# Lynne-Zheng-Linfang/HS-Pose

Measured on AMD Instinct MI355X. Metric: point-clouds/sec (N=1028) HS-layer fwd+bwd, higher is better.
Workload: dtype f32; 1 GPU; HS stack (FaceRecon backbone -> feat) fwd+bwd, B=16/GPU N=1028 fp32, train-mode BN, random-init weights (BASELINE configs[1] shape); global_batch=16, points=1028, parallelism=dp1, hipgraph=True, split_graph=False, grad_exchange=none

## Files before the change

hs_pose_amd/csrc/gather.hip:

```cpp
#include "common.h"
#include "colsum_cloud.h"
#include <type_traits>

namespace hsp {

template <typename FT>
__device__ __forceinline__ void gather_max_rows(const FT* __restrict__ fb, const int32_t* __restrict__ nb, int k,
                                                int C, float4& best, int& a0, int& a1, int& a2, int& a3) {
    constexpr int NB = 8;
    int cur[NB], nxt[NB];
#pragma unroll
    for (int u = 0; u < NB; ++u) cur[u] = nb[min(u, k - 1)];
    for (int n0 = 0; n0 < k; n0 += NB) {
#pragma unroll
        for (int u = 0; u < NB; ++u) nxt[u] = nb[min(n0 + NB + u, k - 1)];
        float4 f[NB];
#pragma unroll
        for (int u = 0; u < NB; ++u) f[u] = Feat<FT>::ld4(fb + (size_t)cur[u] * C);
#pragma unroll
        for (int u = 0; u < NB; ++u) {
            const int n = n0 + u;
            if (n < k) {
                if (f[u].x > best.x) { best.x = f[u].x; a0 = n; }
                if (f[u].y > best.y) { best.y = f[u].y; a1 = n; }
// ... 288 lines not shown
            for (int l = 1; l < RL; ++l) { const float4 v = red[q][l * cq + g]; a.x += v.x; a.y += v.y; a.z += v.z; a.w += v.w; }
            *reinterpret_cast<float4*>(part + (((size_t)b * nchunk + chunk) * 4 + q) * C + (g << 2)) = a;
        }
    }
}

template <bool XYZ>
__global__ __launch_bounds__(1024) void colsum_cloud_kernel(const float* __restrict__ x, const float* __restrict__ xyz, int N, int C,
                                                            int nchunk, int rows, float* __restrict__ out) {
    extern __shared__ float4 cc_smem[];
    colsum_cloud_body<XYZ, 1024, 1>(cc_smem, (int)blockIdx.x, (int)blockIdx.y, x, xyz, N, C, nchunk, rows, out);
}

__global__ __launch_bounds__(256) void colsum_partial_scalar_kernel(const float* __restrict__ x, int N, int C,
                                                                    float* __restrict__ part, int nchunk, int rows) {
    __shared__ float red[256];
    const int tid = threadIdx.x;
    const int RL = 256 / C;
    const int col = tid % C, rl = tid / C;
    const int b = blockIdx.y, chunk = blockIdx.x;
    const int r0 = chunk * rows, r1 = min(N, r0 + rows);
    float s = 0.f;
    if (rl < RL)
        for (int i = r0 + rl; i < r1; i += RL) s += x[((size_t)b * N + i) * C + col];
    red[tid] = s;
    __syncthreads();
    if (rl == 0) {
        for (int l = 1; l < RL; ++l) s += red[l * C + col];
        part[((size_t)b * nchunk + chunk) * C + col] = s;
    }
}

struct ConcatSeg { const void* src; const int32_t* idx; int width; int kind; int nsrc; int col0; };
struct ConcatDesc { ConcatSeg seg[8]; int nseg; int even; int q0[9]; };

template <typename FT>
__global__ __launch_bounds__(256) void concat_rows_kernel(ConcatDesc d, int B, int N, int W, FT* __restrict__ out) {
    using Pair = typename std::conditional<sizeof(FT) == 4, float2, unsigned>::type;
    const long long rows = (long long)B * N;
    if (d.even == 2) {
        const int lane = threadIdx.x & 63;
        const int total = d.q0[d.nseg];
        for (long long row = (long long)blockIdx.x * 4 + (threadIdx.x >> 6); row < rows; row += (long long)gridDim.x * 4) {
            const int b = (int)(row / N);
            FT* o = out + (size_t)row * W;
            for (int q = lane; q < total; q += 64) {
                int sgi = 0;
                while (q >= d.q0[sgi + 1]) ++sgi;
                const ConcatSeg sg = d.seg[sgi];
                const int c = q - d.q0[sgi];
                if (sg.kind >= 2) {
                    const float* ps = reinterpret_cast<const float*>(sg.src);
                    Feat<FT>::st(o + sg.col0 + c, sg.kind == 2 ? ps[(size_t)b * sg.width + c] : ((long long)ps[b] == c ? 1.f : 0.f));
                    continue;
                }
                const FT* src = reinterpret_cast<const FT*>(sg.src);
                src += sg.kind == 0 ? (size_t)row * sg.width : ((size_t)b * sg.nsrc + sg.idx[row]) * sg.width;
                reinterpret_cast<uint4*>(o + sg.col0)[c] = reinterpret_cast<const uint4*>(src)[c];
            }
            const int used = d.seg[d.nseg - 1].col0 + d.seg[d.nseg - 1].width;
            if (lane < W - used) Feat<FT>::st(o + used + lane, 0.f);
        }
        return;
    }
    for (long long row = blockIdx.x; row < rows; row += gridDim.x) {
        const int b = (int)(row / N);
        FT* o = out + (size_t)row * W;
        for (int s = 0; s < d.nseg; ++s) {
            const ConcatSeg sg = d.seg[s];
            if (sg.kind >= 2) {
                const float* src = reinterpret_cast<const float*>(sg.src);
                for (int c = threadIdx.x; c < sg.width; c += 256)
                    Feat<FT>::st(o + sg.col0 + c, sg.kind == 2 ? src[(size_t)b * sg.width + c] : ((long long)src[b] == c ? 1.f : 0.f));
                continue;
            }
            const FT* src = reinterpret_cast<const FT*>(sg.src);
            if (sg.kind == 0) src += (size_t)row * sg.width;
            else src += ((size_t)b * sg.nsrc + sg.idx[row]) * sg.width;
            if (d.even) {
                const Pair* s2 = reinterpret_cast<const Pair*>(src);
                Pair* o2 = reinterpret_cast<Pair*>(o + sg.col0);
                for (int c = threadIdx.x; c < (sg.width >> 1); c += 256) o2[c] = s2[c];
            } else {
                for (int c = threadIdx.x; c < sg.width; c += 256) o[sg.col0 + c] = src[c];
            }
        }
    }
}

__global__ __launch_bounds__(256) void gather_max_bwd_kernel(const float* __restrict__ gout, int gbcast,
                                                             const int32_t* __restrict__ idx,
                                                             const int32_t* __restrict__ qsel, int qstride,
                                                             const uint8_t* __restrict__ argmax, int B, int Nsrc,
                                                             int Nidx, int Nq, int kstride, int C,
                                                             float* __restrict__ gfeat) {
    const int cq = C >> 2;
    const long long total = (long long)B * Nq * cq;
// ... 509 lines not shown
extern "C" int hsp_gather_rows_fwd(const float* feat, const int32_t* idx, int idx_shared, int B, int Nsrc, int Nq,
                                   int C, float* out, int out_stride, hspStream_t stream) {
    if (!feat || !idx || !out || B <= 0 || Nsrc <= 0 || Nq <= 0 || C <= 0 || out_stride < C) return HSP_ERR_BAD_ARG;
    hipStream_t st = as_stream(stream);
    if ((C & 3) == 0) {
        const long long total = (long long)B * Nq * (C >> 2);
        hipLaunchKernelGGL(gather_rows_fwd_kernel, dim3(stream_grid(total)), dim3(256), 0, st, feat, idx, idx_shared, B,
                           Nsrc, Nq, C, out, out_stride);
    } else {
        const long long total = (long long)B * Nq * C;
        hipLaunchKernelGGL(gather_rows_fwd_scalar_kernel, dim3(stream_grid(total)), dim3(256), 0, st, feat, idx,
                           idx_shared, B, Nsrc, Nq, C, out, out_stride);
    }
    return check_launch();
}

extern "C" int hsp_gather_rows_bwd(const float* grad_out, int grad_stride, const int32_t* idx, int idx_shared, int B,
                                   int Nsrc, int Nq, int C, float* grad_feat, hspStream_t stream) {
    if (!grad_out || !idx || !grad_feat || B <= 0 || Nsrc <= 0 || Nq <= 0 || C <= 0 || grad_stride < C)
        return HSP_ERR_BAD_ARG;
    hipStream_t st = as_stream(stream);
    if ((C & 3) == 0 && (grad_stride & 1) == 0 && (reinterpret_cast<uintptr_t>(grad_out) & 7) == 0)
        if (const int tc = pick_scatter_cols(Nsrc, C))
            return launch_scatter_tile<1, float>(tc, grad_out, nullptr, grad_stride, 0, idx, idx_shared, nullptr, 0, nullptr, B,
                                                 Nsrc, Nq, Nq, 1, C, grad_feat, 0, nullptr, st);
    hipError_t e = hipMemsetAsync(grad_feat, 0, (size_t)B * Nsrc * C * sizeof(float), st);
    if (e != hipSuccess) { set_last_hip_error(e); return HSP_ERR_LAUNCH; }
    const long long total = (long long)B * Nq * C;
    hipLaunchKernelGGL(gather_rows_bwd_kernel, dim3(stream_grid(total)), dim3(256), 0, st, grad_out, grad_stride, idx,
                       idx_shared, B, Nsrc, Nq, C, grad_feat);
    return check_launch();
}

template <typename FT, int VEC>
__device__ __forceinline__ void grow_ld(const FT* __restrict__ p, float (&v)[VEC]) {
    if constexpr (sizeof(FT) == 4 && VEC == 2) {
        const float2 t = *reinterpret_cast<const float2*>(p);
        v[0] = t.x; v[1] = t.y;
    } else if constexpr (sizeof(FT) == 4) {
        const float4 t = *reinterpret_cast<const float4*>(p);
        v[0] = t.x; v[1] = t.y; v[2] = t.z; v[3] = t.w;
    } else if constexpr (VEC == 2) {
        const unsigned w = *reinterpret_cast<const unsigned*>(p);
        v[0] = __uint_as_float(w << 16); v[1] = __uint_as_float(w & 0xffff0000u);
    } else {
        const uint2 w = *reinterpret_cast<const uint2*>(p);
        v[0] = __uint_as_float(w.x << 16); v[1] = __uint_as_float(w.x & 0xffff0000u);
        v[2] = __uint_as_float(w.y << 16); v[3] = __uint_as_float(w.y & 0xffff0000u);
    }
}
template <typename FT, int VEC>
__device__ __forceinline__ void grow_st(FT* __restrict__ p, const float (&v)[VEC]) {
    if constexpr (sizeof(FT) == 4 && VEC == 2) {
        *reinterpret_cast<float2*>(p) = make_float2(v[0], v[1]);
    } else if constexpr (sizeof(FT) == 4) {
        *reinterpret_cast<float4*>(p) = make_float4(v[0], v[1], v[2], v[3]);
    } else if constexpr (VEC == 2) {
        *reinterpret_cast<unsigned*>(p) = f32_to_bf16_bits(v[0]) | (f32_to_bf16_bits(v[1]) << 16);
    } else {
        *reinterpret_cast<uint2*>(p) = make_uint2(f32_to_bf16_bits(v[0]) | (f32_to_bf16_bits(v[1]) << 16),
                                                  f32_to_bf16_bits(v[2]) | (f32_to_bf16_bits(v[3]) << 16));
    }
}

template <typename FT, int VEC>
__device__ __forceinline__ void gather_rows_bwd_csr_body(const int bid, const FT* __restrict__ gout, int gstride,
                                                         const int32_t* __restrict__ rev_off,
                                                         const int32_t* __restrict__ rev_edge, int B, int Nsrc, int Nq, int C,
                                                         FT* __restrict__ gfeat) {
    const int cols = C / VEC;
    const int tpr = cols < 256 ? cols : 256;
    const int RB = 256 / tpr;
    const int rl = threadIdx.x / tpr, t = threadIdx.x - rl * tpr;
    const long long row = (long long)bid * RB + rl;
    if (rl >= RB || row >= (long long)B * Nsrc) return;
    const int m = (int)(row % Nsrc), b = (int)(row / Nsrc);
    const int32_t* off = rev_off + (size_t)b * (Nsrc + 1);
    const int32_t* edge = rev_edge + (size_t)b * Nq;
    const int o0 = off[m], o1 = off[m + 1];
    const FT* gb = gout + (size_t)b * Nq * gstride;
    for (int p = t; p < cols; p += tpr) {
        float acc[VEC];
#pragma unroll
        for (int c = 0; c < VEC; ++c) acc[c] = 0.f;
        int e = o0;
        for (; e + 8 <= o1; e += 8) {
            float v[8][VEC];
#pragma unroll
            for (int u = 0; u < 8; ++u) grow_ld<FT, VEC>(gb + (size_t)edge[e + u] * gstride + VEC * p, v[u]);
// ... 16 lines not shown
        grow_st<FT, VEC>(gfeat + (size_t)row * C + VEC * p, acc);
    }
}

template <typename FT>
__global__ __launch_bounds__(256) void gather_rows_bwd_csr_kernel(const FT* __restrict__ gout, int gstride,
                                                                  const int32_t* __restrict__ rev_off,
                                                                  const int32_t* __restrict__ rev_edge, int B,
                                                                  int Nsrc, int Nq, int C,
                                                                  FT* __restrict__ gfeat) {
    gather_rows_bwd_csr_body<FT, 2>((int)blockIdx.x, gout, gstride, rev_off, rev_edge, B, Nsrc, Nq, C, gfeat);
}

struct GatherBwdSeg {
    const void* gout; const int32_t* rev_off; const int32_t* rev_edge; void* gfeat;
    int gstride, nsrc, nq, width, vec;
};
struct GatherBwdDesc { GatherBwdSeg seg[4]; int first[5]; int nseg; };

template <typename FT>
__global__ __launch_bounds__(256) void gather_rows_bwd_csr_multi_kernel(const GatherBwdDesc d, int B) {
    const int bid = (int)blockIdx.x;
    int s = 0;
    while (s + 1 < d.nseg && bid >= d.first[s + 1]) ++s;
    const GatherBwdSeg sg = d.seg[s];
    const FT* gout = reinterpret_cast<const FT*>(sg.gout);
    FT* gfeat = reinterpret_cast<FT*>(sg.gfeat);
    if (sg.vec == 4)
        gather_rows_bwd_csr_body<FT, 4>(bid - d.first[s], gout, sg.gstride, sg.rev_off, sg.rev_edge, B, sg.nsrc, sg.nq, sg.width, gfeat);
    else
        gather_rows_bwd_csr_body<FT, 2>(bid - d.first[s], gout, sg.gstride, sg.rev_off, sg.rev_edge, B, sg.nsrc, sg.nq, sg.width, gfeat);
}

template <typename FT>
static bool gather_bwd_csr_vec_ok(int VEC, const FT* grad_out, int grad_stride, int C, const FT* grad_feat) {
    if ((C % VEC) || (grad_stride % VEC)) return false;
    const size_t al = (size_t)VEC * sizeof(FT) - 1;
    if ((reinterpret_cast<uintptr_t>(grad_out) & al) || (VEC > 2 && (reinterpret_cast<uintptr_t>(grad_feat) & al))) return false;
    const int cols = C / VEC;
    return 256 % (cols < 256 ? cols : 256) == 0;
}

template <typename FT>
static int gather_rows_bwd_csr_impl(const FT* grad_out, int grad_stride, const int32_t* rev_off,
                                    const int32_t* rev_edge, int B, int Nsrc, int Nq, int C, FT* grad_feat,
                                    hspStream_t stream) {
    if (!grad_out || !rev_off || !rev_edge || !grad_feat || B <= 0 || Nsrc <= 0 || Nq <= 0 || C <= 0 || grad_stride < C)
        return HSP_ERR_BAD_ARG;
    if (!gather_bwd_csr_vec_ok<FT>(2, grad_out, grad_stride, C, grad_feat))
        return HSP_ERR_UNSUPPORTED;
    const int tpr = (C >> 1) < 256 ? (C >> 1) : 256;
    const int RB = 256 / tpr;
    const long long rows = (long long)B * Nsrc;
    hipLaunchKernelGGL(gather_rows_bwd_csr_kernel<FT>, dim3((unsigned)((rows + RB - 1) / RB)), dim3(256), 0, as_stream(stream),
                       grad_out, grad_stride, rev_off, rev_edge, B, Nsrc, Nq, C, grad_feat);
    return check_launch();
}

template <typename FT>
static int gather_rows_bwd_csr_multi_impl(int nseg, const FT* const* grad_out, int grad_stride, const int32_t* const* rev_off,
                                          const int32_t* const* rev_edge, int B, const int* Nsrc, int Nq, const int* C,
                                          FT* const* grad_feat, hspStream_t stream) {
    if (nseg <= 0 || nseg > 4 || !grad_out || !rev_off || !rev_edge || !Nsrc || !C || !grad_feat || B <= 0 || Nq <= 0)
        return HSP_ERR_BAD_ARG;
    for (int s = 0; s < nseg; ++s)
        if (!grad_out[s] || !rev_off[s] || !rev_edge[s] || !grad_feat[s] || Nsrc[s] <= 0 || C[s] <= 0 || grad_stride < C[s])
            return HSP_ERR_BAD_ARG;
    int order[4] = {0, 1, 2, 3};
    for (int i = 1; i < nseg; ++i)
        for (int j = i; j > 0 && Nsrc[order[j]] < Nsrc[order[j - 1]]; --j) { const int t = order[j]; order[j] = order[j - 1]; order[j - 1] = t; }
    GatherBwdDesc d;
    d.nseg = nseg;
    long long blocks = 0;
    for (int i = 0; i < nseg; ++i) {
        const int s = order[i];
        if (!gather_bwd_csr_vec_ok<FT>(2, grad_out[s], grad_stride, C[s], grad_feat[s])) return HSP_ERR_UNSUPPORTED;
        const int vec = gather_bwd_csr_vec_ok<FT>(4, grad_out[s], grad_stride, C[s], grad_feat[s]) ? 4 : 2;
        const int cols = C[s] / vec;
        const int RB = 256 / (cols < 256 ? cols : 256);
        d.seg[i] = GatherBwdSeg{grad_out[s], rev_off[s], rev_edge[s], grad_feat[s], grad_stride, Nsrc[s], Nq, C[s], vec};
        d.first[i] = (int)blocks;
        blocks += ((long long)B * Nsrc[s] + RB - 1) / RB;
        if (blocks > 0x7fffffffLL) return HSP_ERR_UNSUPPORTED;
    }
    d.first[nseg] = (int)blocks;
    hipLaunchKernelGGL(gather_rows_bwd_csr_multi_kernel<FT>, dim3((unsigned)blocks), dim3(256), 0, as_stream(stream), d, B);
    return check_launch();
}
extern "C" int hsp_gather_rows_bwd_csr_multi(int nseg, const float* const* grad_out, int grad_stride,
                                             const int32_t* const* rev_off, const int32_t* const* rev_edge, int B,
                                             const int* Nsrc, int Nq, const int* C, float* const* grad_feat, hspStream_t stream) {
    return gather_rows_bwd_csr_multi_impl<float>(nseg, grad_out, grad_stride, rev_off, rev_edge, B, Nsrc, Nq, C, grad_feat, stream);
}
extern "C" int hsp_gather_rows_bwd_csr_multi_bf16(int nseg, const hsp_bf16_t* const* grad_out, int grad_stride,
                                                  const int32_t* const* rev_off, const int32_t* const* rev_edge, int B,
                                                  const int* Nsrc, int Nq, const int* C, hsp_bf16_t* const* grad_feat,
                                                  hspStream_t stream) {
    return gather_rows_bwd_csr_multi_impl<bf16_t>(nseg, reinterpret_cast<const bf16_t* const*>(grad_out), grad_stride, rev_off, rev_edge, B,
                                                  Nsrc, Nq, C, reinterpret_cast<bf16_t* const*>(grad_feat), stream);
}
extern "C" int hsp_gather_rows_bwd_csr(const float* grad_out, int grad_stride, const int32_t* rev_off,
                                       const int32_t* rev_edge, int B, int Nsrc, int Nq, int C, float* grad_feat,
                                       hspStream_t stream) {
    return gather_rows_bwd_csr_impl<float>(grad_out, grad_stride, rev_off, rev_edge, B, Nsrc, Nq, C, grad_feat, stream);
}
extern "C" int hsp_gather_rows_bwd_csr_bf16(const hsp_bf16_t* grad_out, int grad_stride, const int32_t* rev_off,
                                            const int32_t* rev_edge, int B, int Nsrc, int Nq, int C, hsp_bf16_t* grad_feat,
                                            hspStream_t stream) {
    return gather_rows_bwd_csr_impl<bf16_t>(grad_out, grad_stride, rev_off, rev_edge, B, Nsrc, Nq, C, grad_feat, stream);
}
// ... 206 lines not shown

extern "C" int hsp_colsum_rows_bf16(const hsp_bf16_t* x, int B, int N, int C, float* out, void* ws, size_t ws_bytes,
                                    hspStream_t stream) {
    if (!x || !out || B <= 0 || N <= 0 || C <= 0) return HSP_ERR_BAD_ARG;
    if (!colsum_vec4(C)) return HSP_ERR_UNSUPPORTED;
    if (!ws || ws_bytes < hsp_orl_workspace_bytes(B, N, C)) return HSP_ERR_WORKSPACE;
    hipStream_t st = as_stream(stream);
    const int rows = chunk_rows(B, N, C);
    const int nchunk = (N + rows - 1) / rows;
    float* part = reinterpret_cast<float*>(ws);
    hipLaunchKernelGGL(colsum_partial_kernel<bf16_t>, dim3(nchunk, B), dim3(256), 0, st, x, N, C, part, nchunk, rows);
    hipLaunchKernelGGL(chunk_fold_kernel, dim3((B * C + 255) / 256), dim3(256), 0, st, part, B, nchunk, C, 1.0f, out);
    return check_launch();
}

template <typename FT>
static int concat_rows_impl(int nseg, const void* const* src, const int32_t* const* idx, const int* width,
                            const int* kind, const int* nsrc, int B, int N, FT* out, int out_pitch, hspStream_t stream) {
    if (nseg <= 0 || nseg > 8 || !src || !width || !kind || !out || B <= 0 || N <= 0) return HSP_ERR_BAD_ARG;
    ConcatDesc d;
    d.nseg = nseg;
    int col = 0;
    for (int s = 0; s < nseg; ++s) {
        if (!src[s] || width[s] <= 0 || kind[s] < 0 || kind[s] > 3 || (kind[s] == 1 && (!idx || !idx[s]))) return HSP_ERR_BAD_ARG;
        d.seg[s].src = src[s];
        d.seg[s].idx = idx ? idx[s] : nullptr;
        d.seg[s].width = width[s];
        d.seg[s].kind = kind[s];
        d.seg[s].nsrc = nsrc ? nsrc[s] : 0;
        d.seg[s].col0 = col;
        col += width[s];
    }
    if (out_pitch < col) return HSP_ERR_BAD_ARG;
    d.even = (out_pitch & 1) ? 0 : 1;
    for (int s = 0; s < nseg; ++s)
        if (kind[s] < 2 && ((width[s] & 1) || (d.seg[s].col0 & 1) || (reinterpret_cast<uintptr_t>(src[s]) & (2 * sizeof(FT) - 1))))
            d.even = 0;
    if (reinterpret_cast<uintptr_t>(out) & (2 * sizeof(FT) - 1)) d.even = 0;
    if (d.even) {
        constexpr int EP = 16 / (int)sizeof(FT);
        bool q = (out_pitch % EP) == 0 && (reinterpret_cast<uintptr_t>(out) & 15) == 0;
        for (int s = 0; s < nseg && q; ++s)
            if (kind[s] < 2 && ((width[s] % EP) || (d.seg[s].col0 % EP) || (reinterpret_cast<uintptr_t>(src[s]) & 15))) q = false;
        if (q) {
            d.even = 2;
            int acc = 0;
            for (int s = 0; s < nseg; ++s) { d.q0[s] = acc; acc += kind[s] >= 2 ? width[s] : width[s] / EP; }
            d.q0[nseg] = acc;
        }
    }
    const long long rows = (long long)B * N;
    int grid = (int)(rows < 8192 ? rows : 8192);
    if (d.even == 2) grid = (int)((rows + 3) / 4 < 8192 ? (rows + 3) / 4 : 8192);
    hipLaunchKernelGGL(concat_rows_kernel<FT>, dim3(grid), dim3(256), 0, as_stream(stream), d, B, N, out_pitch, out);
    return check_launch();
}
extern "C" int hsp_concat_rows(int nseg, const float* const* src, const int32_t* const* idx, const int* width,
                               const int* kind, const int* nsrc, int B, int N, float* out, hspStream_t stream) {
    int col = 0;
    for (int s = 0; s < nseg && s < 8 && width; ++s) col += width[s];
    return concat_rows_impl<float>(nseg, reinterpret_cast<const void* const*>(src), idx, width, kind, nsrc, B, N, out, col, stream);
}
extern "C" int hsp_concat_rows_pitched(int nseg, const float* const* src, const int32_t* const* idx, const int* width,
                                       const int* kind, const int* nsrc, int B, int N, float* out, int out_pitch,
                                       hspStream_t stream) {
    return concat_rows_impl<float>(nseg, reinterpret_cast<const void* const*>(src), idx, width, kind, nsrc, B, N, out, out_pitch, stream);
}
extern "C" int hsp_concat_rows_bf16(int nseg, const void* const* src, const int32_t* const* idx, const int* width,
                                    const int* kind, const int* nsrc, int B, int N, hsp_bf16_t* out, int out_pitch,
                                    hspStream_t stream) {
    return concat_rows_impl<bf16_t>(nseg, src, idx, width, kind, nsrc, B, N, out, out_pitch, stream);
}

extern "C" int hsp_add_relu_bwd(const float* ga, int lda, const float* gb, int ldb, const float* y, int R, int C, float* out,
                                hspStream_t stream) {
    if (!ga || !y || !out || R <= 0 || C <= 0 || lda < C || (gb && ldb < C)) return HSP_ERR_BAD_ARG;
    if ((C & 1) || (lda & 1) || (gb && (ldb & 1)) || (reinterpret_cast<size_t>(ga) & 7) || (reinterpret_cast<size_t>(gb) & 7))
        return HSP_ERR_UNSUPPORTED;
    const long long total2 = (long long)R * (C >> 1);
    hipLaunchKernelGGL(add_relu_bwd_kernel, dim3(stream_grid(total2)), dim3(256), 0, as_stream(stream), ga, lda, gb, ldb, y, total2,
                       C >> 1, out);
    return check_launch();
}

extern "C" int hsp_residual_bias(float* out, const float* f, const float* t, int B, int N, int C, hspStream_t stream) {
    if (!out || !f || !t || B <= 0 || N <= 0 || C <= 0) return HSP_ERR_BAD_ARG;
    if (C & 3) return HSP_ERR_UNSUPPORTED;
// ... 6 lines not shown
```

hs_pose_amd/csrc/gemm_x3.hip:

```cpp
#include "common.h"
#include <stdlib.h>
#include <type_traits>

namespace hsp {

using f32x16 = __attribute__((ext_vector_type(16))) float;
using bf16x8 = __attribute__((ext_vector_type(8))) __bf16;
using u32x4 = __attribute__((ext_vector_type(4))) unsigned;

struct X3Args {
    const float* A[2];
    const unsigned short* P[2];
    int lda[2], ldp[2], K[2];
    long long ps[2];
    float* C; int ldc;
    int M, N;
    const float* bias;
    const float* resid; int ldr;
    const float* cbias; int rpc;
    float alpha;
    int tiles_m, tiles_n, nsplit;
    float* ws;
    float* bn_shift;
    float* bn_part;
// ... 422 lines not shown
    }
#pragma unroll
    for (int r0 = 0; r0 < 16; r0 += 4) {
        if (it & 1) store4(acc2[0], t - R, it > 0, r0);
        else store4(acc2[1], t - R, it > 0, r0);
    }
}

__global__ __launch_bounds__(256) void gemm_x3_reduce_kernel(const float* __restrict__ ws, int nsplit, long long total, int N,
                                                             float alpha, float* __restrict__ C, int ldc) {
    if ((N & 3) == 0 && (ldc & 3) == 0) {
        const long long total4 = total >> 2;
        const int N4 = N >> 2;
        for (long long e = (long long)blockIdx.x * 256 + threadIdx.x; e < total4; e += (long long)gridDim.x * 256) {
            float4 s = reinterpret_cast<const float4*>(ws)[e];
            for (int sp = 1; sp < nsplit; ++sp) {
                const float4 v = reinterpret_cast<const float4*>(ws)[(size_t)sp * total4 + e];
                s.x += v.x; s.y += v.y; s.z += v.z; s.w += v.w;
            }
            const long long row = e / N4;
            const int c4 = (int)(e - row * N4);
            *reinterpret_cast<float4*>(C + (size_t)row * ldc + 4 * c4) = make_float4(alpha * s.x, alpha * s.y, alpha * s.z, alpha * s.w);
        }
    } else {
        for (long long e = (long long)blockIdx.x * 256 + threadIdx.x; e < total; e += (long long)gridDim.x * 256) {
            float s = ws[e];
            for (int sp = 1; sp < nsplit; ++sp) s += ws[(size_t)sp * total + e];
            const long long row = e / N;
            C[(size_t)row * ldc + (int)(e - row * N)] = alpha * s;
        }
    }
}

__global__ __launch_bounds__(256) void split_params_x3_kernel(const HspSplitDesc* __restrict__ tab, int n) {
    __shared__ float tile[64][33];
    int e = 0;
    while (e + 1 < n && (int)blockIdx.x >= tab[e + 1].tile0) ++e;
    const HspSplitDesc d = tab[e];
    const int t = (int)blockIdx.x - d.tile0;
    const int Nn = d.transpose ? d.cols : d.rows, Kk = d.transpose ? d.rows : d.cols;
    const int tk = (Kk + 63) >> 6;
    const int n0 = (t / tk) * 32, k0 = (t % tk) * 64;
    const int lx = threadIdx.x & 31, ly = threadIdx.x >> 5;
    unsigned* dst = reinterpret_cast<unsigned*>(d.dst);
    float x0[4], x1[4];
    if (d.transpose) {
#pragma unroll
        for (int j = 0; j < 8; ++j) {
            const int k = k0 + ly + 8 * j, nn = n0 + lx;
            tile[ly + 8 * j][lx] = (k < Kk && nn < Nn) ? d.src[(size_t)k * d.ld + nn] : 0.f;
        }
        __syncthreads();
#pragma unroll
        for (int j = 0; j < 4; ++j) { x0[j] = tile[2 * lx][ly + 8 * j]; x1[j] = tile[2 * lx + 1][ly + 8 * j]; }
    } else {
#pragma unroll
        for (int j = 0; j < 4; ++j) {
            const int nn = n0 + ly + 8 * j, k = k0 + 2 * lx;
            const float* p = d.src + (size_t)min(nn, Nn - 1) * d.ld;
            x0[j] = (nn < Nn && k < Kk) ? p[k] : 0.f;
            x1[j] = (nn < Nn && k + 1 < Kk) ? p[k + 1] : 0.f;
        }
    }
#pragma unroll
    for (int j = 0; j < 4; ++j) {
        const int nn = n0 + ly + 8 * j, k = k0 + 2 * lx;
        if (nn >= Nn || k >= Kk) continue;
        float r1[2], r2[2];
        const float xs[2] = {x0[j], x1[j]};
#pragma unroll
        for (int q = 0; q < 2; ++q) {
            const float h = __uint_as_float(__float_as_uint(xs[q]) & 0xffff0000u);
            r1[q] = xs[q] - h;
            const float m = __uint_as_float(__float_as_uint(r1[q]) & 0xffff0000u);
            r2[q] = r1[q] - m;
        }
        const size_t o = ((size_t)nn * d.kp + k) >> 1;
        const size_t psd = (size_t)d.ps >> 1;
        dst[o] = __builtin_amdgcn_perm(__float_as_uint(xs[1]), __float_as_uint(xs[0]), 0x07060302u);
        dst[psd + o] = __builtin_amdgcn_perm(__float_as_uint(r1[1]), __float_as_uint(r1[0]), 0x07060302u);
        dst[2 * psd + o] = __builtin_amdgcn_perm(__float_as_uint(r2[1]), __float_as_uint(r2[0]), 0x07060302u);
    }
}

static int x3_pick_split(long long tiles, int TT) {
    constexpr int per_cu = 2;
    if (tiles >= 2 * HSP_NUM_CU || TT < 16) return 1;
    int ns = (int)((per_cu * HSP_NUM_CU + tiles - 1) / tiles);
    if (ns > TT / 8) ns = TT / 8;
    if (ns > 16) ns = 16;
    if (ns < 2) return 1;
    const int per = (TT + ns - 1) / ns;
    return (TT + per - 1) / per;
}

static int x3_pick_wm(int M, int N) {
    const long long t128 = (long long)((M + 127) / 128) * ((N + X3_BN - 1) / X3_BN);
    return t128 >= 2 * HSP_NUM_CU ? 2 : 1;
}

static int x3_panel_slots(int M, int N, int K1, bool two, int epi0, bool bn, int ldc) {
    if (bn || two || epi0 > 1 || K1 != 128 || N % 128 != 0 || (long long)(M + 32) * ldc * 4 >= (1ll << 31)) return 0;
    const int P = N / 128;
    const int R = (2 * HSP_NUM_CU / P) / HSP_NUM_XCD * HSP_NUM_XCD;
    const int nt = (M + 31) / 32;
    const int rounds = R ? (nt + R - 1) / R : 0;
    return (R && rounds >= 3 && (double)nt / ((double)rounds * R) >= 0.75) ? R : 0;
}

struct X3Plan { int panel_R, wm, TT, ns; };
static X3Plan x3_plan_of(int M, int N, int K1, int K2, int epi, bool bn, bool bn_out, int ldc) {
    X3Plan p;
    p.panel_R = x3_panel_slots(M, N, K1, K2 > 0, epi, bn, ldc);
    p.wm = bn_out ? 1 : x3_pick_wm(M, N);
// ... 484 lines not shown
```

include/hsp.h:

```cpp
#ifndef HSP_H_
#define HSP_H_

#include <stddef.h>
#include <stdint.h>

#ifdef __cplusplus
extern "C" {
#endif

#define HSP_OK 0
#define HSP_ERR_BAD_ARG (-1)
#define HSP_ERR_UNSUPPORTED (-2)
#define HSP_ERR_WORKSPACE (-3)
#define HSP_ERR_LAUNCH (-4)

#define HSP_MAX_K 32

typedef void *hspStream_t;
typedef uint16_t hsp_bf16_t;

int hsp_version(void);
const char *hsp_error_string(int code);
const char *hsp_last_hip_error(void);

// ... 83 lines not shown
int hsp_points_max_bwd(const float *grad_out, const int32_t *argrow, int B, int N, int C, float *grad_x,
                       hspStream_t stream);

size_t hsp_orl_workspace_bytes(int B, int N, int C);
long long hsp_orl_counts_offset(int B, int N, int k, int kstride, int C, size_t ws_bytes);
int hsp_orl_global_fwd(const float *feat, const int32_t *idx, int B, int N, int k, int kstride, int C,
                       float *fg, uint8_t *argmax, void *ws, size_t ws_bytes, hspStream_t stream);
size_t hsp_orl_exact_workspace_bytes(int B, int N, int C);
int hsp_orl_global_exact_f32(const float *feat, const int32_t *idx, int B, int N, int k, int kstride, int C, float *fg,
                             uint8_t *argmax, void *ws, size_t ws_bytes, hspStream_t stream);
int hsp_bn_eval_f32(const float *x, long long R, int C, const float *running_mean, const float *running_var,
                    const float *invstd, const float *weight, const float *bias, float eps, int relu, float *y,
                    hspStream_t stream);
int hsp_layer_out_exact_f32(const float *F, int ldf, const float *Wa, int ldwa, const float *fg, int ldfg, const float *Wb,
                            int ldwb, const float *cloud_t, int two_chain, const float *ste, int ldste, const float *xyz3,
                            const float *w3, int relu, int M, int C, int rows_per_cloud, float *out, int ldo,
                            hspStream_t stream);
int hsp_colsum_rows(const float *x, int B, int N, int C, float *out, void *ws, size_t ws_bytes,
                    hspStream_t stream);

int hsp_add_relu_bwd(const float *ga, int lda, const float *gb, int ldb, const float *y, int R, int C, float *out,
                     hspStream_t stream);
int hsp_residual_bias(float *out, const float *f, const float *t, int B, int N, int C, hspStream_t stream);

int hsp_concat_rows(int nseg, const float *const *src, const int32_t *const *idx, const int *width,
                    const int *kind, const int *nsrc, int B, int N, float *out, hspStream_t stream);

int hsp_gather_rows_fwd(const float *feat, const int32_t *idx, int idx_shared, int B, int Nsrc, int Nq,
                        int C, float *out, int out_stride, hspStream_t stream);
int hsp_gather_rows_bwd(const float *grad_out, int grad_stride, const int32_t *idx, int idx_shared, int B,
                        int Nsrc, int Nq, int C, float *grad_feat, hspStream_t stream);
int hsp_gather_rows_bwd_csr(const float *grad_out, int grad_stride, const int32_t *rev_off, const int32_t *rev_edge,
                            int B, int Nsrc, int Nq, int C, float *grad_feat, hspStream_t stream);
int hsp_gather_rows_bwd_csr_multi(int nseg, const float *const *grad_out, int grad_stride, const int32_t *const *rev_off,
                                  const int32_t *const *rev_edge, int B, const int *Nsrc, int Nq, const int *C,
                                  float *const *grad_feat, hspStream_t stream);

int hsp_gemm_rows_f32(const float *A1, int lda1, const float *B1, int ldb1, int b1_layout, int K1,
                      const float *A2, int lda2, const float *B2, int ldb2, int b2_layout, int K2, int M, int N,
                      const float *bias, const float *resid, int ldr, const float *cloud_bias, int rows_per_cloud,
                      float alpha, const float *xyz3, const float *w3, float *C, int ldc, void *ws, size_t ws_bytes,
                      hspStream_t stream);
size_t hsp_gemm_rows_workspace_bytes(int M, int N, int K1, int K2, int elem_bytes);
int hsp_gemm_rows_plan(int M, int N, int K1, int K2, int elem_bytes, int align, int *out);
int hsp_gemm_rows_bf16(const hsp_bf16_t *A1, int lda1, const hsp_bf16_t *B1, int ldb1, int K1,
                       const hsp_bf16_t *A2, int lda2, const hsp_bf16_t *B2, int ldb2, int K2, int M, int N,
                       const float *bias, const hsp_bf16_t *resid, int ldr, const float *cloud_bias,
                       int rows_per_cloud, float alpha, const float *xyz3, const float *w3, void *C, int ldc,
                       int c_is_f32 ,
                       void *ws, size_t ws_bytes, hspStream_t stream);

int hsp_gemm_wave_supported(int M, int N, int K1, int K2, int cfg);
int hsp_gemm_wave_plan_info(int M, int N, int K1, int K2, int cfg, int *out);
int hsp_gemm_wave_f32(const float *A1, int lda1, const float *B1, int ldb1, int b1_layout, int K1,
                      const float *A2, int lda2, const float *B2, int ldb2, int b2_layout, int K2, int M, int N,
                      const float *bias, const float *resid, int ldr, const float *cloud_bias, int rows_per_cloud,
                      float alpha, const float *xyz3, const float *w3, float *C, int ldc, int cfg, hspStream_t stream);

typedef struct HspSplitDesc { const float *src; void *dst; int rows, cols, ld, transpose, kp, tile0; long long ps; } HspSplitDesc;
int hsp_split_params_x3(const HspSplitDesc *table_dev, int n, int total_tiles, hspStream_t stream);
int hsp_gemm_x3_supported(int M, int N, int K1, int K2);
size_t hsp_gemm_x3_workspace_bytes(int M, int N, int K1, int K2);
int hsp_gemm_x3_plan(int M, int N, int K1, int K2, int epi, int ldc, int *out);
int hsp_gemm_x3_f32(const float *A1, int lda1, const hsp_bf16_t *P1, int ldp1, long long ps1, int K1,
                    const float *A2, int lda2, const hsp_bf16_t *P2, int ldp2, long long ps2, int K2, int M, int N,
                    const float *bias, const float *resid, int ldr, const float *cloud_bias, int rows_per_cloud,
// ... 324 lines not shown
```

Before: 10230 point-clouds/sec.

## Rewrite concat fast path, vectorize split-params packing, relax CSR bwd vector checks

Replaces the 16-byte concat path with a templated kernel that precomputes segment tables in shared memory, software-pipelines row loads against stores, shares gather indices across lanes with shuffles, and uses nontemporal stores. The grid is sized to the CU count. The split_params_x3 kernel now finds its table entry with a wave ballot instead of a serial scan and packs eight elements per thread into 16-byte stores across the three bf16 planes. The CSR backward vector-eligibility check is relaxed to allow 8-byte-aligned float4 loads, and a new plan API is exported. These cut memory-bound concat and packing overheads at the cost of much more complex code and per-U template instantiations.

```diff
diff --git a/hs_pose_amd/csrc/gather.hip b/hs_pose_amd/csrc/gather.hip
--- a/hs_pose_amd/csrc/gather.hip
+++ b/hs_pose_amd/csrc/gather.hip
@@ -344,37 +344,135 @@
 }
 
 struct ConcatSeg { const void* src; const int32_t* idx; int width; int kind; int nsrc; int col0; };
-struct ConcatDesc { ConcatSeg seg[8]; int nseg; int even; int q0[9]; };
-
-template <typename FT>
+struct ConcatDesc { ConcatSeg seg[8]; int nseg; int even; int q0[9]; int t0[9]; int used; };
+
+template <typename FT, int U>
+__device__ __forceinline__ void concat_rows16_body(const ConcatDesc& d, int B, int N, int W, FT* __restrict__ out) {
+    __shared__ uint4 ctab[8], rtab[8];
+    const unsigned pitchb = (unsigned)W * (unsigned)sizeof(FT);
+    char* const outb = reinterpret_cast<char*>(out);
+    if (threadIdx.x == 0) {
+#pragma unroll
+        for (int s = 0; s < 8; ++s) {
+            const bool cp = d.seg[s].kind < 2;
+            const unsigned q16 = 16u * (unsigned)d.q0[s];
+            const uintptr_t sb = reinterpret_cast<uintptr_t>(d.seg[s].src) - (cp ? q16 : 0u);
+            const uintptr_t ib = reinterpret_cast<uintptr_t>(d.seg[s].idx);
+            ctab[s] = cp ? make_uint4((unsigned)sb, (unsigned)(sb >> 32), (unsigned)d.seg[s].width * (unsigned)sizeof(FT),
+                                      (unsigned)d.seg[s].col0 * (unsigned)sizeof(FT) - q16)
+                         : make_uint4((unsigned)sb, (unsigned)(sb >> 32), (unsigned)d.seg[s].width, (unsigned)d.seg[s].col0);
+            rtab[s] = make_uint4((unsigned)ib, (unsigned)(ib >> 32), cp ? (unsigned)d.seg[s].nsrc : (unsigned)d.t0[s], (unsigned)d.seg[s].kind);
+        }
+    }
+    __syncthreads();
+    typedef unsigned u4_t __attribute__((ext_vector_type(4)));
+    typedef __attribute__((address_space(1))) const u4_t* gld_t;
+    typedef __attribute__((address_space(1))) const int32_t* gidx_t;
+    typedef __attribute__((address_space(1))) const float* gf32_t;
+    const int lane = threadIdx.x & 63;
+    const long long rows = (long long)B * N;
+    const long long stride = (long long)gridDim.x * 4;
+    const long long row0 = (long long)blockIdx.x * 4 + __builtin_amdgcn_readfirstlane(threadIdx.x >> 6);
+    if (row0 >= rows) return;
+    const int nrow = (int)((rows - row0 + stride - 1) / stride);
+    const int nseg = d.nseg, used = d.used, total = d.q0[d.nseg], ttotal = d.t0[d.nseg];
+    const unsigned long long outa = reinterpret_cast<uintptr_t>(outb);
+    unsigned long long idx_base = outa;
+    unsigned idx_step = 0;
+    int my_nsrc = 0;
+    bool my_res = false;
+    {
+        const uint4 r = rtab[lane & 7];
+        if (lane < nseg && r.w == 1u) {
+            my_res = true;
+            idx_base = (unsigned long long)r.x | ((unsigned long long)r.y << 32);
+            idx_step = 4;
+            my_nsrc = (int)r.z;
+        }
+    }
+    auto idx_of = [&](long long r) __attribute__((always_inline)) -> int {
+        return *reinterpret_cast<gidx_t>(idx_base + (unsigned long long)idx_step * (unsigned long long)r);
+    };
+    auto resolved = [&](long long r, int iv) __attribute__((always_inline)) -> int {
+        return my_res ? ((int)r / N) * my_nsrc + iv : (int)r;
+    };
+    unsigned long long tl_base = outa;
+    unsigned tl_step = 0, tl_ooff = 0;
+    int tl_c = 0, tl_kind = 0;
+    if (lane < ttotal) {
+        int sg = 0;
+#pragma unroll
+        for (int s = 1; s < 9; ++s) sg += lane >= d.t0[s] ? 1 : 0;
+        const uint4 e = ctab[sg];
+        tl_kind = (int)rtab[sg].w;
+        tl_c = lane - (int)rtab[sg].z;
+        tl_ooff = (e.w + (unsigned)tl_c) * (unsigned)sizeof(FT);
+        tl_base = ((unsigned long long)e.x | ((unsigned long long)e.y << 32)) + (tl_kind == 2 ? 4u * (unsigned)tl_c : 0u);
+        tl_step = tl_kind == 2 ? 4u * e.z : 4u;
+    }
+    for (int qb = 0; qb == 0 || (U == 6 && qb < total); qb += 64 * U) {
+        const bool first = qb == 0;
+        unsigned long long sbase[U];
+        unsigned sstep[U], ooff[U];
+        int sl[U];
+#pragma unroll
+        for (int u = 0; u < U; ++u) {
+            const int q = min(qb + lane + 64 * u, total - 1);
+            int sg = 0;
+#pragma unroll
+            for (int s = 1; s < 9; ++s) sg += q >= d.q0[s] ? 1 : 0;
+            const uint4 e = ctab[sg];
+            sl[u] = sg;
+            sbase[u] = ((unsigned long long)e.x | ((unsigned long long)e.y << 32)) + 16u * (unsigned)q;
+            sstep[u] = e.z;
+            ooff[u] = e.w + 16u * (unsigned)q;
+        }
+        auto load = [&](u4_t (&v)[U], float& tv, long long r, int iv) __attribute__((always_inline)) {
+            const int sr = resolved(r, iv);
+#pragma unroll
+            for (int u = 0; u < U; ++u)
+                v[u] = *reinterpret_cast<gld_t>(sbase[u] + (unsigned long long)(unsigned)__shfl(sr, sl[u]) * sstep[u]);
+            tv = *reinterpret_cast<gf32_t>(tl_base + (unsigned long long)tl_step * (unsigned)((int)r / N));
+        };
+        auto store = [&](const u4_t (&v)[U], float tv, long long r) __attribute__((always_inline)) {
+            char* o = outb + (size_t)r * pitchb;
+#pragma unroll
+            for (int u = 0; u < U; ++u) __builtin_nontemporal_store(v[u], reinterpret_cast<u4_t*>(o + ooff[u]));
+            if (first) {
+                if (tl_kind) Feat<FT>::st(reinterpret_cast<FT*>(o + tl_ooff), tl_kind == 2 ? tv : ((long long)tv == tl_c ? 1.f : 0.f));
+                if (lane < W - used) Feat<FT>::st(reinterpret_cast<FT*>(o) + used + lane, 0.f);
+            }
+        };
+        long long row = row0;
+        u4_t va[U], vb[U];
+        float ta, tb;
+        load(va, ta, row, idx_of(row));
+        int iv_next = idx_of(min(row + stride, rows - 1));
+        auto step = [&](const u4_t (&cur)[U], float tcur, u4_t (&nxt)[U], float& tnxt) __attribute__((always_inline)) {
+            const long long next = row + stride;
+            const int iv_after = idx_of(min(next + stride, rows - 1));
+            load(nxt, tnxt, next, iv_next);
+            iv_next = iv_after;
+            store(cur, tcur, row);
+            row = next;
+        };
+        for (int i = 1;; i += 2) {
+            if (i >= nrow) { store(va, ta, row); break; }
+            step(va, ta, vb, tb);
+            if (i + 1 >= nrow) { store(vb, tb, row); break; }
+            step(vb, tb, va, ta);
+        }
+    }
+}
+
+template <typename FT, int U>
 __global__ __launch_bounds__(256) void concat_rows_kernel(ConcatDesc d, int B, int N, int W, FT* __restrict__ out) {
+    if constexpr (U > 0) {
+        concat_rows16_body<FT, U>(d, B, N, W, out);
+        return;
+    }
     using Pair = typename std::conditional<sizeof(FT) == 4, float2, unsigned>::type;
     const long long rows = (long long)B * N;
-    if (d.even == 2) {
-        const int lane = threadIdx.x & 63;
-        const int total = d.q0[d.nseg];
-        for (long long row = (long long)blockIdx.x * 4 + (threadIdx.x >> 6); row < rows; row += (long long)gridDim.x * 4) {
-            const int b = (int)(row / N);
-            FT* o = out + (size_t)row * W;
-            for (int q = lane; q < total; q += 64) {
-                int sgi = 0;
-                while (q >= d.q0[sgi + 1]) ++sgi;
-                const ConcatSeg sg = d.seg[sgi];
-                const int c = q - d.q0[sgi];
-                if (sg.kind >= 2) {
-                    const float* ps = reinterpret_cast<const float*>(sg.src);
-                    Feat<FT>::st(o + sg.col0 + c, sg.kind == 2 ? ps[(size_t)b * sg.width + c] : ((long long)ps[b] == c ? 1.f : 0.f));
-                    continue;
-                }
-                const FT* src = reinterpret_cast<const FT*>(sg.src);
-                src += sg.kind == 0 ? (size_t)row * sg.width : ((size_t)b * sg.nsrc + sg.idx[row]) * sg.width;
-                reinterpret_cast<uint4*>(o + sg.col0)[c] = reinterpret_cast<const uint4*>(src)[c];
-            }
-            const int used = d.seg[d.nseg - 1].col0 + d.seg[d.nseg - 1].width;
-            if (lane < W - used) Feat<FT>::st(o + used + lane, 0.f);
-        }
-        return;
-    }
     for (long long row = blockIdx.x; row < rows; row += gridDim.x) {
         const int b = (int)(row / N);
         FT* o = out + (size_t)row * W;
@@ -950,19 +1048,23 @@
     return check_launch();
 }
 
+typedef float grow_f4 __attribute__((ext_vector_type(4)));
+typedef unsigned grow_u2 __attribute__((ext_vector_type(2)));
+typedef grow_f4 grow_f4_a8 __attribute__((aligned(8)));
+typedef grow_u2 grow_u2_a4 __attribute__((aligned(4)));
 template <typename FT, int VEC>
 __device__ __forceinline__ void grow_ld(const FT* __restrict__ p, float (&v)[VEC]) {
     if constexpr (sizeof(FT) == 4 && VEC == 2) {
         const float2 t = *reinterpret_cast<const float2*>(p);
         v[0] = t.x; v[1] = t.y;
     } else if constexpr (sizeof(FT) == 4) {
-        const float4 t = *reinterpret_cast<const float4*>(p);
+        const grow_f4 t = *reinterpret_cast<const grow_f4_a8*>(p);
         v[0] = t.x; v[1] = t.y; v[2] = t.z; v[3] = t.w;
     } else if constexpr (VEC == 2) {
         const unsigned w = *reinterpret_cast<const unsigned*>(p);
         v[0] = __uint_as_float(w << 16); v[1] = __uint_as_float(w & 0xffff0000u);
     } else {
-        const uint2 w = *reinterpret_cast<const uint2*>(p);
+        const grow_u2 w = *reinterpret_cast<const grow_u2_a4*>(p);
         v[0] = __uint_as_float(w.x << 16); v[1] = __uint_as_float(w.x & 0xffff0000u);
         v[2] = __uint_as_float(w.y << 16); v[3] = __uint_as_float(w.y & 0xffff0000u);
     }
@@ -972,7 +1074,9 @@
     if constexpr (sizeof(FT) == 4 && VEC == 2) {
         *reinterpret_cast<float2*>(p) = make_float2(v[0], v[1]);
     } else if constexpr (sizeof(FT) == 4) {
-        *reinterpret_cast<float4*>(p) = make_float4(v[0], v[1], v[2], v[3]);
+        grow_f4 t;
+        t.x = v[0]; t.y = v[1]; t.z = v[2]; t.w = v[3];
+        *reinterpret_cast<grow_f4*>(p) = t;
     } else if constexpr (VEC == 2) {
         *reinterpret_cast<unsigned*>(p) = f32_to_bf16_bits(v[0]) | (f32_to_bf16_bits(v[1]) << 16);
     } else {
@@ -1055,13 +1159,21 @@
         gather_rows_bwd_csr_body<FT, 2>(bid - d.first[s], gout, sg.gstride, sg.rev_off, sg.rev_edge, B, sg.nsrc, sg.nq, sg.width, gfeat);
 }
 
-template <typename FT>
-static bool gather_bwd_csr_vec_ok(int VEC, const FT* grad_out, int grad_stride, int C, const FT* grad_feat) {
-    if ((C % VEC) || (grad_stride % VEC)) return false;
-    const size_t al = (size_t)VEC * sizeof(FT) - 1;
-    if ((reinterpret_cast<uintptr_t>(grad_out) & al) || (VEC > 2 && (reinterpret_cast<uintptr_t>(grad_feat) & al))) return false;
+static bool gather_bwd_csr_vec_ok(int VEC, size_t esz, const void* grad_out, int grad_stride, int C, const void* grad_feat) {
+    if ((C % VEC) || (grad_stride % 2)) return false;
+    if (reinterpret_cast<uintptr_t>(grad_out) & (2 * esz - 1)) return false;
+    if (VEC > 2 && (reinterpret_cast<uintptr_t>(grad_feat) & ((size_t)VEC * esz - 1))) return false;
     const int cols = C / VEC;
     return 256 % (cols < 256 ? cols : 256) == 0;
+}
+static int gather_bwd_csr_multi_vec(size_t esz, const void* grad_out, int grad_stride, int C, const void* grad_feat) {
+    if (!gather_bwd_csr_vec_ok(2, esz, grad_out, grad_stride, C, grad_feat)) return 0;
+    return gather_bwd_csr_vec_ok(4, esz, grad_out, grad_stride, C, grad_feat) ? 4 : 2;
+}
+extern "C" int hsp_gather_rows_bwd_csr_multi_plan(const void* grad_out, int grad_stride, int C, const void* grad_feat,
+                                                  int elem_bytes) {
+    if (!grad_out || !grad_feat || C <= 0 || grad_stride < C || (elem_bytes != 4 && elem_bytes != 2)) return HSP_ERR_BAD_ARG;
+    return gather_bwd_csr_multi_vec((size_t)elem_bytes, grad_out, grad_stride, C, grad_feat);
 }
 
 template <typename FT>
@@ -1070,7 +1182,7 @@
                                     hspStream_t stream) {
     if (!grad_out || !rev_off || !rev_edge || !grad_feat || B <= 0 || Nsrc <= 0 || Nq <= 0 || C <= 0 || grad_stride < C)
         return HSP_ERR_BAD_ARG;
-    if (!gather_bwd_csr_vec_ok<FT>(2, grad_out, grad_stride, C, grad_feat))
+    if (!gather_bwd_csr_vec_ok(2, sizeof(FT), grad_out, grad_stride, C, grad_feat))
         return HSP_ERR_UNSUPPORTED;
     const int tpr = (C >> 1) < 256 ? (C >> 1) : 256;
     const int RB = 256 / tpr;
@@ -1097,8 +1209,8 @@
     long long blocks = 0;
     for (int i = 0; i < nseg; ++i) {
         const int s = order[i];
-        if (!gather_bwd_csr_vec_ok<FT>(2, grad_out[s], grad_stride, C[s], grad_feat[s])) return HSP_ERR_UNSUPPORTED;
-        const int vec = gather_bwd_csr_vec_ok<FT>(4, grad_out[s], grad_stride, C[s], grad_feat[s]) ? 4 : 2;
+        const int vec = gather_bwd_csr_multi_vec(sizeof(FT), grad_out[s], grad_stride, C[s], grad_feat[s]);
+        if (!vec) return HSP_ERR_UNSUPPORTED;
         const int cols = C[s] / vec;
         const int RB = 256 / (cols < 256 ? cols : 256);
         d.seg[i] = GatherBwdSeg{grad_out[s], rev_off[s], rev_edge[s], grad_feat[s], grad_stride, Nsrc[s], Nq, C[s], vec};
@@ -1371,6 +1483,7 @@
         col += width[s];
     }
     if (out_pitch < col) return HSP_ERR_BAD_ARG;
+    d.used = col;
     d.even = (out_pitch & 1) ? 0 : 1;
     for (int s = 0; s < nseg; ++s)
         if (kind[s] < 2 && ((width[s] & 1) || (d.seg[s].col0 & 1) || (reinterpret_cast<uintptr_t>(src[s]) & (2 * sizeof(FT) - 1))))
@@ -1378,20 +1491,38 @@
     if (reinterpret_cast<uintptr_t>(out) & (2 * sizeof(FT) - 1)) d.even = 0;
     if (d.even) {
         constexpr int EP = 16 / (int)sizeof(FT);
-        bool q = (out_pitch % EP) == 0 && (reinterpret_cast<uintptr_t>(out) & 15) == 0;
+        bool q = (out_pitch % EP) == 0 && (reinterpret_cast<uintptr_t>(out) & 15) == 0 && (long long)B * N <= 0x7fffffffLL;
+        for (int s = 0; s < nseg && q; ++s) if (kind[s] == 1 && (long long)B * d.seg[s].nsrc > 0x7fffffffLL) q = false;
         for (int s = 0; s < nseg && q; ++s)
             if (kind[s] < 2 && ((width[s] % EP) || (d.seg[s].col0 % EP) || (reinterpret_cast<uintptr_t>(src[s]) & 15))) q = false;
-        if (q) {
-            d.even = 2;
-            int acc = 0;
-            for (int s = 0; s < nseg; ++s) { d.q0[s] = acc; acc += kind[s] >= 2 ? width[s] : width[s] / EP; }
-            d.q0[nseg] = acc;
-        }
+        int acc = 0, tacc = 0;
+        for (int s = 0; s < nseg; ++s) {
+            d.q0[s] = acc; d.t0[s] = tacc;
+            if (kind[s] >= 2) tacc += width[s] <= 64 ? width[s] : 65; else acc += width[s] / EP;
+        }
+        for (int s = nseg; s < 9; ++s) { d.q0[s] = s == nseg ? acc : 0x7fffffff; d.t0[s] = s == nseg ? tacc : 0x7fffffff; }
+        if (q && acc > 0 && tacc <= 64) d.even = 2;
     }
     const long long rows = (long long)B * N;
     int grid = (int)(rows < 8192 ? rows : 8192);
-    if (d.even == 2) grid = (int)((rows + 3) / 4 < 8192 ? (rows + 3) / 4 : 8192);
-    hipLaunchKernelGGL(concat_rows_kernel<FT>, dim3(grid), dim3(256), 0, as_stream(stream), d, B, N, out_pitch, out);
+    if (d.even == 2) {
+        const long long wr = (rows + 3) / 4, cap = 8 * HSP_NUM_CU, per = (wr + cap / 2) / cap < 1 ? 1 : (wr + cap / 2) / cap;
+        grid = (int)((wr + per - 1) / per);
+    }
+    int slots = 0;
+    if (d.even == 2) slots = (d.q0[nseg] + 63) / 64 < 1 ? 1 : (d.q0[nseg] + 63) / 64 > 6 ? 6 : (d.q0[nseg] + 63) / 64;
+#define HSP_CONCAT_LAUNCH(U) \
+    hipLaunchKernelGGL((concat_rows_kernel<FT, U>), dim3(grid), dim3(256), 0, as_stream(stream), d, B, N, out_pitch, out)
+    switch (slots) {
+        case 0: HSP_CONCAT_LAUNCH(0); break;
+        case 1: HSP_CONCAT_LAUNCH(1); break;
+        case 2: HSP_CONCAT_LAUNCH(2); break;
+        case 3: HSP_CONCAT_LAUNCH(3); break;
+        case 4: HSP_CONCAT_LAUNCH(4); break;
+        case 5: HSP_CONCAT_LAUNCH(5); break;
+        default: HSP_CONCAT_LAUNCH(6); break;
+    }
+#undef HSP_CONCAT_LAUNCH
     return check_launch();
 }
 extern "C" int hsp_concat_rows(int nseg, const float* const* src, const int32_t* const* idx, const int* width,
diff --git a/hs_pose_amd/csrc/gemm_x3.hip b/hs_pose_amd/csrc/gemm_x3.hip
--- a/hs_pose_amd/csrc/gemm_x3.hip
+++ b/hs_pose_amd/csrc/gemm_x3.hip
@@ -478,54 +478,76 @@
     }
 }
 
+__device__ __forceinline__ int split_entry_of(const HspSplitDesc* __restrict__ tab, int n, int bid) {
+    const int lane = threadIdx.x & 63;
+    int cnt = 0;
+    for (int e0 = 0; e0 < n; e0 += 64) {
+        const int e = e0 + lane;
+        const bool le = e < n && tab[min(e, n - 1)].tile0 <= bid;
+        cnt += __popcll(__ballot(le));
+    }
+    return cnt > 0 ? cnt - 1 : 0;
+}
+
 __global__ __launch_bounds__(256) void split_params_x3_kernel(const HspSplitDesc* __restrict__ tab, int n) {
     __shared__ float tile[64][33];
-    int e = 0;
-    while (e + 1 < n && (int)blockIdx.x >= tab[e + 1].tile0) ++e;
-    const HspSplitDesc d = tab[e];
+    const HspSplitDesc d = tab[split_entry_of(tab, n, (int)blockIdx.x)];
     const int t = (int)blockIdx.x - d.tile0;
     const int Nn = d.transpose ? d.cols : d.rows, Kk = d.transpose ? d.rows : d.cols;
     const int tk = (Kk + 63) >> 6;
     const int n0 = (t / tk) * 32, k0 = (t % tk) * 64;
-    const int lx = threadIdx.x & 31, ly = threadIdx.x >> 5;
+    const int nn = n0 + (int)(threadIdx.x >> 3), k = k0 + 8 * (int)(threadIdx.x & 7);
+    float x[8];
+    if (d.transpose) {
+        const int lx = threadIdx.x & 31, ly = threadIdx.x >> 5;
+#pragma unroll
+        for (int j = 0; j < 8; ++j) {
+            const int kk = k0 + ly + 8 * j, nc = n0 + lx;
+            tile[ly + 8 * j][lx] = (kk < Kk && nc < Nn) ? d.src[(size_t)kk * d.ld + nc] : 0.f;
+        }
+        __syncthreads();
+#pragma unroll
+        for (int q = 0; q < 8; ++q) x[q] = tile[8 * (threadIdx.x & 7) + q][threadIdx.x >> 3];
+    } else {
+        const float* p = d.src + (size_t)min(nn, Nn - 1) * d.ld;
+        if (k + 8 <= Kk && !(d.ld & 3) && !(reinterpret_cast<uintptr_t>(d.src) & 15)) {
+            const float4 a = *reinterpret_cast<const float4*>(p + k), b = *reinterpret_cast<const float4*>(p + k + 4);
+            x[0] = a.x; x[1] = a.y; x[2] = a.z; x[3] = a.w; x[4] = b.x; x[5] = b.y; x[6] = b.z; x[7] = b.w;
+        } else {
+#pragma unroll
+            for (int q = 0; q < 8; ++q) x[q] = k + q < Kk ? p[k + q] : 0.f;
+        }
+    }
+    if (nn >= Nn || k >= Kk) return;
+    unsigned w[3][4];
+#pragma unroll
+    for (int q = 0; q < 4; ++q) {
+        float r1[2], r2[2];
+#pragma unroll
+        for (int u = 0; u < 2; ++u) {
+            const float h = __uint_as_float(__float_as_uint(x[2 * q + u]) & 0xffff0000u);
+            r1[u] = x[2 * q + u] - h;
+            const float m = __uint_as_float(__float_as_uint(r1[u]) & 0xffff0000u);
+            r2[u] = r1[u] - m;
+        }
+        w[0][q] = __builtin_amdgcn_perm(__float_as_uint(x[2 * q + 1]), __float_as_uint(x[2 * q]), 0x07060302u);
+        w[1][q] = __builtin_amdgcn_perm(__float_as_uint(r1[1]), __float_as_uint(r1[0]), 0x07060302u);
+        w[2][q] = __builtin_amdgcn_perm(__float_as_uint(r2[1]), __float_as_uint(r2[0]), 0x07060302u);
+    }
     unsigned* dst = reinterpret_cast<unsigned*>(d.dst);
-    float x0[4], x1[4];
-    if (d.transpose) {
-#pragma unroll
-        for (int j = 0; j < 8; ++j) {
-            const int k = k0 + ly + 8 * j, nn = n0 + lx;
-            tile[ly + 8 * j][lx] = (k < Kk && nn < Nn) ? d.src[(size_t)k * d.ld + nn] : 0.f;
-        }
-        __syncthreads();
-#pragma unroll
-        for (int j = 0; j < 4; ++j) { x0[j] = tile[2 * lx][ly + 8 * j]; x1[j] = tile[2 * lx + 1][ly + 8 * j]; }
+    const size_t o = ((size_t)nn * d.kp + k) >> 1;
+    const size_t psd = (size_t)d.ps >> 1;
+    if (k + 8 <= Kk && !(d.kp & 7) && !(d.ps & 7) && !(reinterpret_cast<uintptr_t>(d.dst) & 15)) {
+#pragma unroll
+        for (int pl = 0; pl < 3; ++pl)
+            *reinterpret_cast<uint4*>(dst + pl * psd + o) = make_uint4(w[pl][0], w[pl][1], w[pl][2], w[pl][3]);
     } else {
 #pragma unroll
-        for (int j = 0; j < 4; ++j) {
-            const int nn = n0 + ly + 8 * j, k = k0 + 2 * lx;
-            const float* p = d.src + (size_t)min(nn, Nn - 1) * d.ld;
-            x0[j] = (nn < Nn && k < Kk) ? p[k] : 0.f;
-            x1[j] = (nn < Nn && k + 1 < Kk) ? p[k + 1] : 0.f;
-        }
-    }
-#pragma unroll
-    for (int j = 0; j < 4; ++j) {
-        const int nn = n0 + ly + 8 * j, k = k0 + 2 * lx;
-        if (nn >= Nn || k >= Kk) continue;
-        float r1[2], r2[2];
-        const float xs[2] = {x0[j], x1[j]};
-#pragma unroll
-        for (int q = 0; q < 2; ++q) {
-            const float h = __uint_as_float(__float_as_uint(xs[q]) & 0xffff0000u);
-            r1[q] = xs[q] - h;
-            const float m = __uint_as_float(__float_as_uint(r1[q]) & 0xffff0000u);
-            r2[q] = r1[q] - m;
-        }
-        const size_t o = ((size_t)nn * d.kp + k) >> 1;
-        const size_t psd = (size_t)d.ps >> 1;
-        dst[o] = __builtin_amdgcn_perm(__float_as_uint(xs[1]), __float_as_uint(xs[0]), 0x07060302u);
-        dst[psd + o] = __builtin_amdgcn_perm(__float_as_uint(r1[1]), __float_as_uint(r1[0]), 0x07060302u);
-        dst[2 * psd + o] = __builtin_amdgcn_perm(__float_as_uint(r2[1]), __float_as_uint(r2[0]), 0x07060302u);
+        for (int q = 0; q < 4; ++q)
+            if (k + 2 * q < Kk) {
+#pragma unroll
+                for (int pl = 0; pl < 3; ++pl) dst[pl * psd + o + q] = w[pl][q];
+            }
     }
 }
 
diff --git a/include/hsp.h b/include/hsp.h
--- a/include/hsp.h
+++ b/include/hsp.h
@@ -139,6 +139,7 @@
                         int Nsrc, int Nq, int C, float *grad_feat, hspStream_t stream);
 int hsp_gather_rows_bwd_csr(const float *grad_out, int grad_stride, const int32_t *rev_off, const int32_t *rev_edge,
                             int B, int Nsrc, int Nq, int C, float *grad_feat, hspStream_t stream);
+int hsp_gather_rows_bwd_csr_multi_plan(const void *grad_out, int grad_stride, int C, const void *grad_feat, int elem_bytes);
 int hsp_gather_rows_bwd_csr_multi(int nseg, const float *const *grad_out, int grad_stride, const int32_t *const *rev_off,
                                   const int32_t *const *rev_edge, int B, const int *Nsrc, int Nq, const int *C,
                                   float *const *grad_feat, hspStream_t stream);
```

Result: no change. 10330 point-clouds/sec, median of 6 (+0.9%).
